# tier4/icp_rust

Hardware: AMD Instinct MI355X
Metric: ICP iterations/sec on 1M-pt 3D pair (higher is better)
Workload: dtype f64

## Files before the change

### icp_rust_amd/csrc/gn_device.hpp

```cpp
#pragma once
#include "common.hpp"

namespace icp {

__device__ __forceinline__ unsigned long long f2k(double v) {
  const unsigned long long u = (unsigned long long)__double_as_longlong(v);
  return (u >> 63) ? ~u : (u | 0x8000000000000000ull);
}
__device__ __forceinline__ double k2f(unsigned long long k) {
  const unsigned long long u = (k >> 63) ? (k & 0x7fffffffffffffffull) : ~k;
  return __longlong_as_double((long long)u);
}

__device__ __forceinline__ int pass_shift(int pass) { return pass < 5 ? 52 - 12 * pass : 0; }
__device__ __forceinline__ int pass_bits(int pass) { return pass < 5 ? 12 : 4; }

__device__ __forceinline__ double huber_rho(double e) {
  const double k = ICP_HUBER_K;
  const double k2 = k * k;
  return (e <= k2) ? e : (2. * k * __dsqrt_rn(e) - k2);
}
__device__ __forceinline__ double huber_drho(double e) {
  const double k = ICP_HUBER_K;
  const double k2 = k * k;
// ... 224 lines not shown
      accumulate_pair<true>(s[u], r0[u], r1[u], T, acc);
    }
  }
}

template <int SCOPE = __HIP_MEMORY_SCOPE_AGENT>
__device__ __forceinline__ void fold_block_sums(const double *partials, int blocks, double *s_tot) {
  double tot[kNSum + 1];
#pragma unroll
  for (int k = 0; k < kNSum + 1; ++k) tot[k] = 0.;
  for (int i = threadIdx.x; i < blocks; i += kReduceThreads) {
    double v[kNSum];
#pragma unroll
    for (int k = 0; k < kNSum; ++k)
      v[k] = __hip_atomic_load(&partials[(size_t)i * (kNSum + 1) + k], __ATOMIC_RELAXED, SCOPE);
#pragma unroll
    for (int k = 0; k < kNSum; ++k) tot[k] = tot[k] + v[k];
  }
  block_reduce_store<kNSum + 1>(tot, s_tot);
}

template <int SCOPE = __HIP_MEMORY_SCOPE_AGENT>
__device__ __forceinline__ void fold_block_sums_lean(const double *partials, int blocks, double *s_tot) {
  __shared__ double sm[kReduceThreads / 64];
  const int t = threadIdx.x;
  for (int q = 0; q < kNSum; ++q) {
    double v[1] = {0.};
    for (int i = t; i < blocks; i += kReduceThreads)
      v[0] = v[0] + __hip_atomic_load(&partials[(size_t)i * (kNSum + 1) + q], __ATOMIC_RELAXED, SCOPE);
    wave_tree<1>(v);
    if ((t & 63) == 0) sm[t >> 6] = v[0];
    __syncthreads();
    if (t == 0) {
      double s = sm[0];
      for (int w = 1; w < kReduceThreads / 64; ++w) s = s + sm[w];
      s_tot[q] = s;
    }
    __syncthreads();
  }
  if (t == 0) s_tot[kNSum] = 0.;
  __syncthreads();
}

constexpr int kFoldH = (kNSum + 1) / 2;
template <int SCOPE = __HIP_MEMORY_SCOPE_AGENT>
__device__ __forceinline__ void fold256_load(const double *partials, int blocks, double (&x)[kFoldH]) {
  static_assert(kReduceThreads == 512 && (kNSum + 1) == 20 && kReduceMaxBlocks <= 256, "two halves of ten sums, one row per thread");
  const int t = threadIdx.x, row = t & 255, half = t >> 8;
#pragma unroll
  for (int k = 0; k < kFoldH; ++k)
    x[k] = (row < blocks && half * kFoldH + k < kNSum)
               ? __hip_atomic_load(&partials[(size_t)row * (kNSum + 1) + half * kFoldH + k], __ATOMIC_RELAXED, SCOPE)
               : 0.;
}
__device__ __forceinline__ void fold256_reduce(const double (&x)[kFoldH], int blocks, double *s_tot) {
  constexpr int H = kFoldH;
  __shared__ double sm[8][H];
  const int t = threadIdx.x, row = t & 255, lane = t & 63, wave = t >> 6;
  double v[H];
#pragma unroll
  for (int k = 0; k < H; ++k) v[k] = 0.;
  if (row < blocks) {
#pragma unroll
    for (int k = 0; k < H; ++k) v[k] = v[k] + x[k];
  }
  wave_tree<H>(v);
  if (lane == 0) {
#pragma unroll
    for (int k = 0; k < H; ++k) sm[wave][k] = v[k];
  }
  __syncthreads();
  if (t < kNSum + 1) {
    const int h = t / H, k = t % H;
    double s = sm[4 * h][k];
    for (int w = 1; w < 4; ++w) s = s + sm[4 * h + w][k];
    s_tot[t] = s + 0.;
  }
}
constexpr int kFoldQ = kFoldH / 2;
template <int SCOPE = __HIP_MEMORY_SCOPE_AGENT>
__device__ __forceinline__ void fold256_half_load(const double *partials, int blocks, int h, double (&x)[kFoldQ]) {
  static_assert(kFoldQ * 2 == kFoldH, "two quarters per half");
  const int t = threadIdx.x, row = t & 255, c0 = h * kFoldH + (t >> 8) * kFoldQ;
#pragma unroll
  for (int k = 0; k < kFoldQ; ++k)
    x[k] = (row < blocks && c0 + k < kNSum)
               ? __hip_atomic_load(&partials[(size_t)row * (kNSum + 1) + c0 + k], __ATOMIC_RELAXED, SCOPE)
               : 0.;
}
__device__ __forceinline__ void fold256_half_reduce(const double (&x)[kFoldQ], int blocks, double *out) {
  constexpr int Q = kFoldQ;
  __shared__ double sm[8][Q];
  const int t = threadIdx.x, row = t & 255, lane = t & 63, wave = t >> 6;
  double v[Q];
#pragma unroll
  for (int k = 0; k < Q; ++k) v[k] = 0.;
  if (row < blocks) {
#pragma unroll
    for (int k = 0; k < Q; ++k) v[k] = v[k] + x[k];
  }
  wave_tree<Q>(v);
  if (lane == 0) {
#pragma unroll
    for (int k = 0; k < Q; ++k) sm[wave][k] = v[k];
  }
  __syncthreads();
  if (t < kFoldH) {
    const int g = t / Q, k = t % Q;
    double s = sm[4 * g][k];
    for (int w = 1; w < 4; ++w) s = s + sm[4 * g + w][k];
    out[t] = s + 0.;
  }
}

template <int SCOPE = __HIP_MEMORY_SCOPE_AGENT>
__device__ __forceinline__ void fold_block_sums_256(const double *partials, int blocks, double *s_tot) {
  double x[kFoldH];
  fold256_load<SCOPE>(partials, blocks, x);
  fold256_reduce(x, blocks, s_tot);
}

template <int SCOPE = __HIP_MEMORY_SCOPE_AGENT>
__device__ __forceinline__ double fold_one_load(const double *partials, int blocks, int q) {
  const int t = threadIdx.x;
  return (t < 256 && t < blocks && q < kNSum) ? __hip_atomic_load(&partials[(size_t)t * (kNSum + 1) + q], __ATOMIC_RELAXED, SCOPE)
                                               : 0.;
}
__device__ __forceinline__ double fold_one_reduce(double x, int blocks, double *sm4) {
  const int t = threadIdx.x, lane = t & 63, wave = t >> 6;
  double v[1] = {0.};
  if (t < 256 && t < blocks) v[0] = v[0] + x;
  wave_tree<1>(v);
  if (t < 256 && lane == 0) sm4[wave] = v[0];
  __syncthreads();
  double s = sm4[0];
  for (int w = 1; w < 4; ++w) s = s + sm4[w];
  return s + 0.;
}
template <int SCOPE = __HIP_MEMORY_SCOPE_AGENT>
__device__ __forceinline__ double fold_one_sum_256(const double *partials, int blocks, int q, double *sm4) {
  const int t = threadIdx.x, lane = t & 63, wave = t >> 6;
  double v[1] = {0.};
  if (t < 256) {
    const double x = (t < blocks && q < kNSum) ? __hip_atomic_load(&partials[(size_t)t * (kNSum + 1) + q], __ATOMIC_RELAXED, SCOPE) : 0.;
    if (t < blocks) v[0] = v[0] + x;
  }
  wave_tree<1>(v);
  if (t < 256 && lane == 0) sm4[wave] = v[0];
  __syncthreads();
  double s = sm4[0];
  for (int w = 1; w < 4; ++w) s = s + sm4[w];
  return s + 0.;
}

__device__ __forceinline__ void publish_folded(const double *s_tot, GnResult *res, unsigned seq, const double (&sig)[2],
                                               const double (&med)[2], int nan_flag, int overflow) {
  if (threadIdx.x < 64) {
    if (threadIdx.x < kNAcc + 1)
      res->acc[threadIdx.x] = threadIdx.x < kNAcc ? combine_sum(s_tot, (int)threadIdx.x, sig) : 0.;
    if (threadIdx.x == kNAcc + 1) {
      res->sigma[0] = sig[0];
      res->sigma[1] = sig[1];
      res->median[0] = med[0];
      res->median[1] = med[1];
    }
    if (threadIdx.x == kNAcc + 2) {
      res->nan_flag = nan_flag;
      res->overflow = overflow;
    }
    asm volatile("s_waitcnt vmcnt(0)" ::: "memory");
    if (threadIdx.x == 0) __hip_atomic_store(&res->seq, seq, __ATOMIC_RELEASE, __HIP_MEMORY_SCOPE_SYSTEM);
// ... 40 lines not shown
```

### icp_rust_amd/csrc/gn_win.hip

```cpp
#include "common.hpp"
#include "gn_device.hpp"
#include "gn_win_device.hpp"
#include "gn_loop.hpp"

namespace icp {


template <bool SUMS, int BATCH = kWinBatch>
__device__ __forceinline__ void win_hist_body(const double2 *__restrict__ a, const double2 *__restrict__ b,
                                              const Pose &T, double *__restrict__ rx, double *__restrict__ ry,
                                              unsigned n, const WinParams &P, uint32_t *whist, WinState *st,
                                              GnScalars *scal, double *partials, int status_cls = -1) {
  __shared__ uint32_t lh[2 * kWinBins];
  if (SUMS && status_cls >= 0 && blockIdx.x == 0 && threadIdx.x < (unsigned)kShardStatusWords)
    whist[2 * kWinBins + threadIdx.x] = (int)threadIdx.x == status_cls ? 1u : 0u;
  double acc[SUMS ? kNSum : 1];
#pragma unroll
  for (int k = 0; k < (SUMS ? kNSum : 1); ++k) acc[k] = 0.;
#ifdef ICP_WIN_DEBUG
  long long wst[6];
  wst[0] = wall_clock64();
#endif
  for (unsigned i = threadIdx.x; i < 2u * kWinBins; i += kWinThreads) lh[i] = 0;
  __syncthreads();
// ... 747 lines not shown
      __hip_atomic_store(&whist[i], 0u, __ATOMIC_RELAXED, __HIP_MEMORY_SCOPE_AGENT);
    fail = fail || got[0] != sel.med_cnt[0] || got[1] != sel.med_cnt[1] || got[2] != sel.ring_cnt[0] ||
           got[3] != sel.ring_cnt[1];
    const unsigned klo = (n - 1) / 2, khi = n / 2;
    if (!fail) {
      unsigned long long key[2][2];
      const double m_lo[2] = {sel.range[0][0], sel.range[1][0]}, m_hi[2] = {sel.range[0][1], sel.range[1][1]};
      const long long mlo[2] = {(long long)klo - sel.med_base[0], (long long)klo - sel.med_base[1]};
      const long long mhi[2] = {(long long)khi - sel.med_base[0], (long long)khi - sel.med_base[1]};
#ifdef ICP_WIN_DEBUG
      fst[3] = wall_clock64();
#endif
      select_n<2, PM>(vm, sel.med_cnt, m_lo, m_hi, mlo, mhi, key, fail);
#ifdef ICP_WIN_DEBUG
      fst[4] = wall_clock64();
#endif
      if (!fail) {
#pragma unroll
        for (int d = 0; d < 2; ++d) {
          med[d] = middle_of(n, key[d][0], key[d][1]);
#pragma unroll
          for (int u = 0; u < PR; ++u) vr[d][u] = fabs(vr[d][u] - med[d]);
        }
        const double r_lo[2] = {sel.range[0][2], sel.range[1][2]}, r_hi[2] = {sel.range[0][3], sel.range[1][3]};
        const long long dlo[2] = {(long long)klo - sel.inner[0], (long long)klo - sel.inner[1]};
        const long long dhi[2] = {(long long)khi - sel.inner[0], (long long)khi - sel.inner[1]};
        select_n<2, PR>(vr, sel.ring_cnt, r_lo, r_hi, dlo, dhi, key, fail);
        if (!fail) {
          sig[0] = ICP_PPF34 * middle_of(n, key[0][0], key[0][1]);
          sig[1] = ICP_PPF34 * middle_of(n, key[1][0], key[1][1]);
        } else {
          med[0] = med[1] = 0.;
        }
      }
    }
  }
  if (tid == 0 && fail) st->fail = 1u;
  asm volatile("s_waitcnt vmcnt(0)" ::: "memory");
  __syncthreads();
  if (ahead && tid == 0) fill_ahead_pose(s_tot, sig, !fail && !nan_flag, outer, ahead, res);
#ifdef ICP_WIN_DEBUG
  fst[5] = wall_clock64();
#endif
  publish_folded(s_tot, res, seq, sig, med, nan_flag, fail ? 2 : 0);
#ifdef ICP_WIN_DEBUG
  asm volatile("s_waitcnt vmcnt(0)" ::: "memory");
  fst[6] = wall_clock64();
  if (tid == 0 && seq % 16 == 5)
    printf("[F last blk %d of %d] compact %lld ticket %lld loads %lld sel1 %lld sel2 %lld publish %lld (x10ns) cnt %u %u %u %u\n", blockIdx.x,
           gridDim.x, fst[1] - fst[0], fst[2] - fst[1], fst[3] - fst[2], fst[4] - fst[3], fst[5] - fst[4], fst[6] - fst[5],
           sel.med_cnt[0], sel.med_cnt[1], sel.ring_cnt[0], sel.ring_cnt[1]);
#endif
}

struct PickLds {
  union {
    struct {
      uint32_t cum[2 * kWinBins];
      uint32_t med[2][kWinCapMed], ring[2][kWinCapRing];
    } g;
    SelectLds<2> sel;
  };
};

struct PickDimLds {
  union {
    struct {
      uint32_t cum[kWinBins];
      double med[kWinCapMed], ring[kWinCapRing];
    } g;
    SelectLds<1> sel;
  };
};

struct WinBins1 {
  unsigned mlo, mhi, a0, b1, i0, i1;
  bool fail;
};
struct WinSel1 {
  unsigned med_base, med_cnt, inner, ring_cnt;
  double range[4];
};

__device__ __forceinline__ WinBins1 win_resolve_dim(const uint32_t *__restrict__ row, unsigned n, const WinDim &w,
                                                    WinState *st, int d, uint32_t *cum, WinSel1 &sel) {
  __shared__ unsigned s_wtot[kReduceThreads / 64];
  __shared__ int s_j[2], s_t[2], s_rng[7];
  __shared__ unsigned s_selu[4];
  __shared__ double s_seld[4];
  constexpr int PER = kWinBins / kReduceThreads, NW = kReduceThreads / 64;
  static_assert(PER == 4, "one 16-byte load per thread");
  const int tid = threadIdx.x, lane = tid & 63, wave = tid >> 6;
  const unsigned klo = (n - 1) / 2, khi = n / 2;
  if (tid < 2) s_j[tid] = -1;
  const uint4 x = reinterpret_cast<const uint4 *>(row)[tid];
  const unsigned v[PER] = {x.x, x.y, x.z, x.w};
  const unsigned tot = (x.x + x.y) + (x.z + x.w);
  const unsigned inc = wave_scan_inclusive(tot);
  if (lane == 63) s_wtot[wave] = inc;
  __syncthreads();
  {
    unsigned wbase = 0;
#pragma unroll
    for (int q = 0; q < NW; ++q) wbase += (q < wave) ? s_wtot[q] : 0u;
    unsigned run = wbase + inc - tot;
#pragma unroll
    for (int i = 0; i < PER; ++i) {
      cum[PER * tid + i] = run;
      if (run <= klo && klo < run + v[i]) s_j[0] = PER * tid + i;
      if (run <= khi && khi < run + v[i]) s_j[1] = PER * tid + i;
      run += v[i];
    }
  }
  __syncthreads();
  WinGeom geo = {};
  if (wave < 2) {
    geo = window_geometry(cum, n, w, s_j[0], s_j[1]);
    const int t = geo.ok ? bracket_search(cum, n, w, geo, wave) : -1;
    if (lane == 0) s_t[wave] = t;
  }
  __syncthreads();
  if (wave == 0) {
    WinRanges R = {};
    unsigned med_base = 0, med_cnt = 0, inner = 0, ring_cnt = 0;
    double range[4] = {0., 0., 0., 0.};
    unsigned counted = 0;
#pragma unroll
    for (int q = 0; q < NW; ++q) counted += s_wtot[q];
    bool ok = counted == n && resolve_window(cum, n, w, geo, s_t[0], s_t[1], R, med_base, med_cnt, inner, ring_cnt, range);
    if (ok)
      ok = R.mlo >= kF1 && R.mhi < kC1 && R.i0 <= R.i1 && R.a0 >= kF0 && R.i0 - 1 < kC0 && R.i1 + 1 >= kF2 &&
           R.b1 <= kWinBins - 2;
    if (lane == 0) {
      s_rng[0] = R.mlo;
      s_rng[1] = R.mhi;
      s_rng[2] = R.a0;
      s_rng[3] = R.b1;
      s_rng[4] = R.i0;
      s_rng[5] = R.i1;
      s_rng[6] = ok ? 0 : 1;
      s_selu[0] = med_base;
      s_selu[1] = med_cnt;
      s_selu[2] = inner;
      s_selu[3] = ring_cnt;
#pragma unroll
      for (int k = 0; k < 4; ++k) s_seld[k] = range[k];
      if (st) {
        st->med_base[d] = med_base;
        st->med_cnt[d] = med_cnt;
        st->ring_inner[d] = inner;
        st->ring_cnt[d] = ring_cnt;
        st->med_lo[d] = range[0];
        st->med_hi[d] = range[1];
        st->ring_lo[d] = range[2];
        st->ring_hi[d] = range[3];
      }
    }
  }
  __syncthreads();
  WinBins1 B;
  B.mlo = (unsigned)s_rng[0];
  B.mhi = (unsigned)s_rng[1];
  B.a0 = (unsigned)s_rng[2];
  B.b1 = (unsigned)s_rng[3];
  B.i0 = (unsigned)s_rng[4];
  B.i1 = (unsigned)s_rng[5];
  B.fail = s_rng[6] != 0;
  sel.med_base = s_selu[0];
  sel.med_cnt = s_selu[1];
  sel.inner = s_selu[2];
  sel.ring_cnt = s_selu[3];
#pragma unroll
  for (int k = 0; k < 4; ++k) sel.range[k] = s_seld[k];
  return B;
}

struct PickArgs {
  unsigned n;
  WinParams P;
  uint32_t *whist;
  WinState *st;
  const double *seg_all;
  const unsigned short *dir_all;
  int segments;
  GnScalars *scal;
  const double *partials;
  int sum_blocks;
  GnResult *res;
  unsigned seq;
  AheadPose *ahead;
  Pose outer;
  WinJoin *join;
};

__device__ __forceinline__ void win_pick_dim_body(const PickArgs &A, const int d, const bool primary, PickDimLds &L) {
  const unsigned n = A.n;
  WinState *const st = A.st;
  const double *__restrict__ seg_all = A.seg_all;
  const unsigned short *__restrict__ dir_all = A.dir_all;
  WinJoin *const J = A.join;
  constexpr int PM = kWinCapMed / kReduceThreads, PR = kWinCapRing / kReduceThreads;
  static_assert(kReduceMaxBlocks * 2 == kReduceThreads, "two threads per segment");
  __shared__ double s_tot[kNSum + 1];
  __shared__ unsigned s_wcnt[kReduceThreads / 64];
  __shared__ int s_last;
  __shared__ unsigned s_pflags;
  __shared__ double s_pms[2];
  const unsigned tid = threadIdx.x;
#ifdef ICP_WIN_DEBUG
  long long pst[10];
  pst[0] = wall_clock64();
  for (int k = 1; k < 10; ++k) pst[k] = pst[0];
#define PSTAMP(k) pst[k] = wall_clock64()
#else
#define PSTAMP(k)
#endif
  const int nan_flag = __hip_atomic_load(&A.scal->nan_flag, __ATOMIC_RELAXED, __HIP_MEMORY_SCOPE_AGENT);
  const unsigned stage_overflow = __hip_atomic_load(&st->stage_overflow, __ATOMIC_RELAXED, __HIP_MEMORY_SCOPE_AGENT);
  WinSel1 sel;
  const WinBins1 R = win_resolve_dim(A.whist + (size_t)d * kWinBins, n, A.P.d[d], primary ? st : nullptr, d, L.g.cum, sel);
  double fx[kFoldQ];
  fold256_half_load(A.partials, A.sum_blocks, d, fx);
  PSTAMP(1);
  const bool fail = R.fail;
  bool bucket_miss = stage_overflow != 0, sel_fail = false;
  double med = 0., sig = 0.;
  {
    const bool usable = !fail && !bucket_miss;
    constexpr int kPickU = 12;
    const unsigned w = tid & (unsigned)(kReduceMaxBlocks - 1), part = tid / (unsigned)kReduceMaxBlocks;
    const unsigned lane = tid & 63u, wave = tid >> 6;
    unsigned p0 = 0, l0 = 0, p1 = 0, l1 = 0;
    if (usable && (int)w < A.segments) {
      const unsigned short *dir = dir_all + (size_t)w * kBktDir;
      if (part == 0) {
        const unsigned fm = word_to_fine(d, R.mlo), len_m = R.mhi - R.mlo + 1u;
        const unsigned m0 = dir[fm], m_end = dir[fm + len_m];
        p0 = m0;
        l0 = m_end - m0;
      } else {
        const unsigned fa = word_to_fine(d, R.a0), fb = word_to_fine(d, R.i1 + 1u);
        const unsigned len_a = R.i0 - R.a0, len_b = R.b1 - R.i1;
        const unsigned a_beg = dir[fa], a_end = dir[fa + len_a], b_beg = dir[fb], b_end = dir[fb + len_b];
        p0 = a_beg;
        l0 = a_end - a_beg;
        p1 = b_beg;
        l1 = b_end - b_beg;
      }
    }
    const unsigned cnt = l0 + l1;
    const unsigned nld = cnt < (unsigned)kBktStage ? cnt : (unsigned)kBktStage;
    const double *const seg = seg_all + (size_t)w * kBktStage;
    auto member = [&](unsigned k) -> unsigned { return k < l0 ? p0 + k : p1 + (k - l0); };
    double own[kPickU];
#pragma unroll
    for (int u = 0; u < kPickU; ++u) {
      const unsigned at = member((unsigned)u);
      own[u] = ((unsigned)u < nld && at < (unsigned)kBktStage) ? seg[at] : 0.;
    }
    const unsigned inc = wave_scan_inclusive(cnt);
    if (lane == 63u) s_wcnt[wave] = inc;
    __syncthreads();
    PSTAMP(2);
    unsigned before = 0, tot_m = 0, tot_r = 0;
    {
      constexpr unsigned HW = kReduceThreads / 64 / 2;
#pragma unroll
      for (unsigned q = 0; q < 2 * HW; ++q) {
        const unsigned x = s_wcnt[q];
        if (q < HW) tot_m += x;
        else tot_r += x;
        before += (q < wave && (q < HW) == (wave < HW)) ? x : 0u;
      }
    }
    if (usable) bucket_miss = tot_m != sel.med_cnt || tot_r != sel.ring_cnt;
    const bool go = usable && !bucket_miss;
    if (go) {
      double *const vals = part ? L.g.ring : L.g.med;
      const unsigned cap = part ? (unsigned)kWinCapRing : (unsigned)kWinCapMed;
      const unsigned off = before + inc - cnt;
#pragma unroll
      for (int u = 0; u < kPickU; ++u)
        if ((unsigned)u < nld && off + (unsigned)u < cap) vals[off + (unsigned)u] = own[u];
      for (unsigned k = kPickU; k < nld; ++k) {
        const unsigned at = member(k);
        if (at < (unsigned)kBktStage && off + k < cap) vals[off + k] = seg[at];
      }
    }
    __syncthreads();
    double vm[1][PM], vr[1][PR];
#pragma unroll
    for (int u = 0; u < PM; ++u) {
      const unsigned e = tid + u * kReduceThreads;
      vm[0][u] = (go && e < sel.med_cnt) ? L.g.med[e] : 0.;
    }
#pragma unroll
    for (int u = 0; u < PR; ++u) {
      const unsigned e = tid + u * kReduceThreads;
      vr[0][u] = (go && e < sel.ring_cnt) ? L.g.ring[e] : 0.;
    }
    {
      unsigned long long *row = reinterpret_cast<unsigned long long *>(A.whist + (size_t)d * kWinBins);
#pragma unroll
      for (int u = 0; u < kWinBins / 2 / kReduceThreads; ++u)
        __hip_atomic_store(&row[tid + u * kReduceThreads], 0ull, __ATOMIC_RELAXED, __HIP_MEMORY_SCOPE_AGENT);
// ... 2 lines not shown
    __syncthreads();
    PSTAMP(3);
    const unsigned klo = (n - 1) / 2, khi = n / 2;
    if (go) {
      unsigned long long key[1][2];
      const unsigned cm[1] = {sel.med_cnt}, cr[1] = {sel.ring_cnt};
      const double m_lo[1] = {sel.range[0]}, m_hi[1] = {sel.range[1]};
      const long long mlo[1] = {(long long)klo - sel.med_base}, mhi[1] = {(long long)khi - sel.med_base};
      select_n_lds<1, PM>(vm, cm, m_lo, m_hi, mlo, mhi, key, sel_fail, L.sel);
      PSTAMP(4);
      if (!sel_fail) {
        med = middle_of(n, key[0][0], key[0][1]);
#pragma unroll
        for (int u = 0; u < PR; ++u) vr[0][u] = fabs(vr[0][u] - med);
        const double r_lo[1] = {sel.range[2]}, r_hi[1] = {sel.range[3]};
        const long long dlo[1] = {(long long)klo - sel.inner}, dhi[1] = {(long long)khi - sel.inner};
        select_n_lds<1, PR>(vr, cr, r_lo, r_hi, dlo, dhi, key, sel_fail, L.sel);
        PSTAMP(5);
        if (!sel_fail) sig = ICP_PPF34 * middle_of(n, key[0][0], key[0][1]);
      }
    }
  }
  const unsigned flags = (fail ? 1u : 0u) | (bucket_miss ? 2u : 0u) | (sel_fail ? 4u : 0u);
  WinJoinDim *const mine = &J->dim[d];
  if (tid < (unsigned)kFoldH) __hip_atomic_store(&mine->tot[tid], s_tot[d * kFoldH + tid], __ATOMIC_RELAXED, __HIP_MEMORY_SCOPE_AGENT);
  if (tid == 64) {
    __hip_atomic_store(&mine->med, med, __ATOMIC_RELAXED, __HIP_MEMORY_SCOPE_AGENT);
    __hip_atomic_store(&mine->sig, sig, __ATOMIC_RELAXED, __HIP_MEMORY_SCOPE_AGENT);
    __hip_atomic_store(&mine->flags, flags, __ATOMIC_RELAXED, __HIP_MEMORY_SCOPE_AGENT);
  }
  asm volatile("s_waitcnt vmcnt(0)" ::: "memory");
  __syncthreads();
  PSTAMP(6);
  if (tid == 0)
    s_last = (int)(__hip_atomic_fetch_add(&J->ticket, 1u, __ATOMIC_RELAXED, __HIP_MEMORY_SCOPE_AGENT) & 1u);
  __syncthreads();
  if (!s_last) {
#ifdef ICP_WIN_DEBUG
    if (tid == 0 && A.seq % 16 == 5)
      printf("[P%d first] resolve %lld dir+scan %lld place+fold %lld sel1 %lld sel2 %lld store %lld (x10ns) cnt %u %u\n", d,
             pst[1] - pst[0], pst[2] - pst[1], pst[3] - pst[2], pst[4] - pst[3], pst[5] - pst[4], pst[6] - pst[5],
             sel.med_cnt, sel.ring_cnt);
#endif
    return;
  }
  const int o = 1 - d;
  const WinJoinDim *const other = &J->dim[o];
  static_assert(offsetof(WinJoinDim, tot) == 16 && offsetof(WinJoinDim, flags) == 96, "words of the record");
  if (tid < 13) {
    const unsigned long long x =
        __hip_atomic_load(reinterpret_cast<const unsigned long long *>(other) + tid, __ATOMIC_RELAXED, __HIP_MEMORY_SCOPE_AGENT);
    if (tid < 2) s_pms[tid] = __longlong_as_double((long long)x);
    else if (tid < 12) s_tot[o * kFoldH + (tid - 2)] = __longlong_as_double((long long)x);
    else s_pflags = (unsigned)x;
  }
  __syncthreads();
  PSTAMP(7);
  const unsigned all = flags | s_pflags;
  const bool any_fail = (all & 1u) != 0, any_bucket = (all & 2u) != 0;
  const bool failed = any_fail || (!any_bucket && (all & 4u) != 0);
  const bool missed = failed || any_bucket;
  const double m_me = missed ? 0. : med, s_me = missed ? 0. : sig, m_ot = missed ? 0. : s_pms[0], s_ot = missed ? 0. : s_pms[1];
  const double med2[2] = {d ? m_ot : m_me, d ? m_me : m_ot}, sig2[2] = {d ? s_ot : s_me, d ? s_me : s_ot};
  if (tid == 0) {
    if (missed) st->fail = 1u;
    else if (primary) st->fail = 0u;
    if (stage_overflow) __hip_atomic_store(&st->stage_overflow, 0u, __ATOMIC_RELAXED, __HIP_MEMORY_SCOPE_AGENT);
  }
  const int overflow = missed ? (failed ? 2 : 3) : 0;
  GnResult *const res = A.res;
  if (A.ahead) {
    if (tid == 0) fill_ahead_pose(s_tot, sig2, !missed && !nan_flag, A.outer, A.ahead, res);
    publish_values<1>(s_tot, res, sig2, med2, nan_flag, overflow);
    PSTAMP(8);
    __syncthreads();
    publish_seq(res, A.seq);
  } else {
    PSTAMP(8);
    publish_folded(s_tot, res, A.seq, sig2, med2, nan_flag, overflow);
  }
#ifdef ICP_WIN_DEBUG
  asm volatile("s_waitcnt vmcnt(0)" ::: "memory");
  PSTAMP(9);
  if (tid == 0 && A.seq % 16 == 5)
    printf("[P%d last] resolve %lld dir+scan %lld place+fold %lld sel1 %lld sel2 %lld store %lld ticket+loads %lld ahead %lld "
           "publish %lld (x10ns) cnt %u %u\n", d, pst[1] - pst[0], pst[2] - pst[1], pst[3] - pst[2], pst[4] - pst[3],
           pst[5] - pst[4], pst[6] - pst[5], pst[7] - pst[6], pst[8] - pst[7], pst[9] - pst[8], sel.med_cnt, sel.ring_cnt);
#endif
#undef PSTAMP
}

__global__ __launch_bounds__(kReduceThreads) void k_win_pick(PickArgs A) {
  __shared__ PickDimLds L;
  win_pick_dim_body(A, (int)blockIdx.x, true, L);
}

__global__ __launch_bounds__(kWinThreads, 4) void k_win_hist_sums_bkt2(HistBktArgs A, HistBktArgs B) {
  __shared__ HistBktLds S;
  const unsigned half = gridDim.x >> 1;
  if (blockIdx.x < half) win_hist_sums_bkt_body(A, blockIdx.x, half, S);
  else win_hist_sums_bkt_body(B, blockIdx.x - half, half, S);
}
struct PickPairArgs {
  PickArgs e[2];
};
__global__ __launch_bounds__(kReduceThreads) void k_win_pick2(PickPairArgs X) {
  __shared__ PickDimLds L;
  const unsigned second = blockIdx.x >> 1;
  win_pick_dim_body(X.e[second], (int)(blockIdx.x & 1u), second == 0u, L);
}

namespace {
constexpr long long kPipeTimeoutTicks = 300000000;
__device__ __forceinline__ void pst_u32(unsigned *p, unsigned v) { __hip_atomic_store(p, v, __ATOMIC_RELAXED, __HIP_MEMORY_SCOPE_SYSTEM); }
__device__ __forceinline__ void pst_f64(double *p, double v) { __hip_atomic_store(p, v, __ATOMIC_RELAXED, __HIP_MEMORY_SCOPE_SYSTEM); }
__device__ __forceinline__ unsigned pld_u32(const unsigned *p) { return __hip_atomic_load(p, __ATOMIC_RELAXED, __HIP_MEMORY_SCOPE_SYSTEM); }
__device__ __forceinline__ double pld_f64(const double *p) { return __hip_atomic_load(p, __ATOMIC_RELAXED, __HIP_MEMORY_SCOPE_SYSTEM); }

__device__ __forceinline__ bool pipe_poll(const unsigned long long *words, int count, unsigned gen, LoopInbox *const *box, int W,
                                          LoopInbox *me, unsigned *payload_or) {
  __shared__ int s_pok;
  __shared__ unsigned s_ppay;
  if (threadIdx.x < 64) {
    const int lane = (int)threadIdx.x;
    unsigned long long seen = 0;
    int ok = 1;
    const long long t0 = wall_clock64();
    for (;;) {
      bool here = true;
      if (lane < count) {
        seen = __hip_atomic_load(&words[lane], __ATOMIC_RELAXED, __HIP_MEMORY_SCOPE_SYSTEM);
        here = (int)((unsigned)seen - gen) >= 0;
      }
      if (__all(here)) break;
      int stop = 0;
      if (lane == 0) {
        if (pld_u32(&me->abort[0]) != 0u) stop = 1;
        else if (wall_clock64() - t0 > kPipeTimeoutTicks) {
          for (int q = 0; q < W; ++q) pst_u32(&box[q]->abort[0], 1u);
          stop = 1;
        }
      }
      if (__builtin_amdgcn_readfirstlane(stop)) {
        ok = 0;
        break;
      }
      __builtin_amdgcn_s_sleep(1);
    }
    unsigned pay = lane < count ? (unsigned)(seen >> 32) : 0u;
#pragma unroll
    for (int off = 32; off >= 1; off >>= 1) pay |= (unsigned)__shfl_xor((int)pay, off);
    if (lane == 0) {
      s_pok = ok;
      s_ppay = pay;
    }
  }
  __syncthreads();
  *payload_or = s_ppay;
  return s_pok != 0;
}
}

constexpr int kPipeFuse = 8;
struct PickRank {
  uint32_t *whist;
  WinState *st;
  const double *seg_all;
  const unsigned short *dir_all;
  GnScalars *scal;
  const double *partials;
// ... 694 lines not shown
```

### icp_rust_amd/csrc/gn_win_device.hpp

```cpp
#pragma once
#include "common.hpp"
#include "gn_device.hpp"

namespace icp {

constexpr int kWinThreads = 512;
constexpr int kWinBatch = 4;
#ifndef ICP_SELECT_DIRECT
#define ICP_SELECT_DIRECT 256
#endif
constexpr int kSubBins = 1024;
constexpr int kSmallCap = 1024;
constexpr size_t kWinMinN = 1u << 12;
constexpr size_t kWinMaxN = 1u << 22;

constexpr int kF0 = 1, kC0 = kF0 + kWinFine, kF1 = kC0 + kWinCoarse, kC1 = kF1 + kWinFine, kF2 = kC1 + kWinCoarse;
static_assert(kF2 + kWinFine == kWinBins - 1, "bin layout");

__device__ __forceinline__ unsigned region_bin(double off, double scale, int first, int count) {
  const unsigned k = (unsigned)(off * scale);
  return (unsigned)first + (k < (unsigned)count ? k : (unsigned)(count - 1));
}

__device__ __forceinline__ unsigned wbin(double r, const WinDim &w) {
  if (!(r >= w.x[0])) return 0u;
  if (r >= w.x[5]) return (unsigned)(kWinBins - 1);
  if (r < w.x[1]) return region_bin(r - w.x[0], w.sf, kF0, kWinFine);
  if (r < w.x[2]) return region_bin(r - w.x[1], w.sc, kC0, kWinCoarse);
  if (r < w.x[3]) return region_bin(r - w.x[2], w.sf, kF1, kWinFine);
  if (r < w.x[4]) return region_bin(r - w.x[3], w.sc, kC1, kWinCoarse);
  return region_bin(r - w.x[4], w.sf, kF2, kWinFine);
}

__device__ __forceinline__ unsigned wbin_cold(double r, const WinDim &w) {
  const bool g1 = r >= w.x[1], g2 = r >= w.x[2], g3 = r >= w.x[3], g4 = r >= w.x[4];
  const double base = g4 ? w.x[4] : (g3 ? w.x[3] : (g2 ? w.x[2] : (g1 ? w.x[1] : w.x[0])));
  const bool coarse = g1 != g2 || g3 != g4;
  const int first = g4 ? kF2 : (g3 ? kC1 : (g2 ? kF1 : (g1 ? kC0 : kF0)));
  const bool inside = r >= w.x[0] && !(r >= w.x[5]);
  const double off = inside ? r - base : 0.;
  const unsigned j = region_bin(off, coarse ? w.sc : w.sf, first, coarse ? kWinCoarse : kWinFine);
  if (!(r >= w.x[0])) return 0u;
  return r >= w.x[5] ? (unsigned)(kWinBins - 1) : j;
}

struct WinRegion {
  double base, scale;
  unsigned first, last;
  unsigned pad[2];
};
static_assert(sizeof(WinRegion) == 32, "one ds_read_b128 + one ds_read_b64");
__device__ __forceinline__ void win_region_table(const WinDim &w, WinRegion *tab, int r) {
  const bool coarse = r & 1;
  WinRegion e;
  e.base = w.x[r];
  e.scale = coarse ? w.sc : w.sf;
  e.first = (unsigned)(r == 0 ? kF0 : r == 1 ? kC0 : r == 2 ? kF1 : r == 3 ? kC1 : kF2);
  e.last = (unsigned)((coarse ? kWinCoarse : kWinFine) - 1);
  e.pad[0] = e.pad[1] = 0u;
  tab[r] = e;
}
__device__ __forceinline__ unsigned wbin_tab(double r, const WinDim &w, const WinRegion *tab, bool &below, bool &above,
                                             bool &fine) {
  below = !(r >= w.x[0]);
  above = r >= w.x[5];
  const unsigned reg = (unsigned)(r >= w.x[1]) + (unsigned)(r >= w.x[2]) + (unsigned)(r >= w.x[3]) + (unsigned)(r >= w.x[4]);
  const WinRegion e = tab[reg];
  const unsigned k = (unsigned)((r - e.base) * e.scale);
  fine = !(reg & 1u) & !below & !above;
  const unsigned j = e.first + (k < e.last ? k : e.last);
  return below ? 0u : (above ? (unsigned)(kWinBins - 1) : j);
}

__device__ __forceinline__ bool fine_bin(unsigned j) {
  return (j - (unsigned)kF0 < (unsigned)kWinFine) | (j - (unsigned)kF1 < (unsigned)kWinFine) |
         (j - (unsigned)kF2 < (unsigned)kWinFine);
}

__device__ __forceinline__ double wedge(int j, const WinDim &w) {
  if (j >= kWinBins - 1) return w.x[5];
  const bool g1 = j >= kC0, g2 = j >= kF1, g3 = j >= kC1, g4 = j >= kF2;
  const double base = g4 ? w.x[4] : (g3 ? w.x[3] : (g2 ? w.x[2] : (g1 ? w.x[1] : w.x[0])));
  const int first = g4 ? kF2 : (g3 ? kC1 : (g2 ? kF1 : (g1 ? kC0 : kF0)));
  const bool coarse = g1 != g2 || g3 != g4;
  return base + (double)(j - first) / (coarse ? w.sc : w.sf);
}

template <typename F>
__device__ __forceinline__ int wave_last_true(int lo, int hi, F &&pred) {
  const int lane = threadIdx.x & 63;
  int best = lo - 1;
  while (lo <= hi) {
    const int step = (hi - lo + 64) >> 6;
    const int t = lo + lane * step;
    const bool ok = t <= hi && pred(t);
    const int cnt = __popcll(__ballot(ok));
    if (cnt == 0) break;
    best = lo + (cnt - 1) * step;
    const int nhi = best + step - 1 < hi ? best + step - 1 : hi;
    lo = best + 1;
    hi = nhi;
  }
  return best;
}

struct WinRanges {
  int mlo, mhi;
  int a0, b1;
  int i0, i1;
};

struct WinGeom {
  int jlo, jhi;
  double mL, mU, fine, q;
  int tmax;
  bool ok;
};

__device__ __forceinline__ WinGeom window_geometry(const uint32_t *c, unsigned n, const WinDim &w, int jlo_known = -1,
                                                   int jhi_known = -1) {
  auto C = [&](int j) -> unsigned { return j >= kWinBins ? n : c[j]; };
  const unsigned klo = (n - 1) / 2, khi = n / 2;
  WinGeom g;
  if (jlo_known >= 0 && jhi_known >= 0) {
    g.jlo = jlo_known;
    g.jhi = jhi_known;
  } else {
    g.jlo = wave_last_true(0, kWinBins - 1, [&](int j) { return c[j] <= klo; });
    g.jhi = (C(g.jlo + 1) > khi) ? g.jlo : wave_last_true(0, kWinBins - 1, [&](int j) { return c[j] <= khi; });
  }
  g.ok = !(g.jlo < 1 || g.jhi > kWinBins - 2);
  g.mL = g.ok ? wedge(g.jlo, w) : 0.;
  g.mU = g.ok ? wedge(g.jhi + 1, w) : 0.;
  g.fine = 1. / w.sf;
  g.q = 0.25 * g.fine;
  g.tmax = (int)((w.x[5] - w.x[0]) * w.sf) + 2;
  return g;
}

__device__ __forceinline__ void inside_bins(const WinGeom &g, const WinDim &w, double d, int &s, int &e) {
  s = (int)wbin_cold(g.mU - d + g.q, w) + 1;
  e = (int)wbin_cold(g.mL + d - g.q, w);
}
__device__ __forceinline__ void possible_bins(const WinGeom &g, const WinDim &w, double d, int &s, int &e) {
  s = (int)wbin_cold(g.mL - d - g.q, w);
  e = (int)wbin_cold(g.mU + d + g.q, w) + 1;
}

__device__ __forceinline__ int bracket_search(const uint32_t *c, unsigned n, const WinDim &w, const WinGeom &g,
                                              int role) {
  auto C = [&](int j) -> unsigned { return j >= kWinBins ? n : c[j]; };
  const unsigned klo = (n - 1) / 2, khi = n / 2;
  if (role == 0)
    return wave_last_true(0, g.tmax, [&](int t) {
      int s, e;
      possible_bins(g, w, (double)t * g.fine, s, e);
      return C(e) - C(s) <= klo;
    });
  return wave_last_true(0, g.tmax, [&](int t) {
           int s, e;
           inside_bins(g, w, (double)t * g.fine, s, e);
           return (s < e ? C(e) - C(s) : 0u) <= khi;
         }) + 1;
}

__device__ __forceinline__ bool resolve_window(const uint32_t *c, unsigned n, const WinDim &w, const WinGeom &g,
                                               int t1, int t2, WinRanges &R, unsigned &med_base,
                                               unsigned &med_cnt, unsigned &inner, unsigned &ring_cnt,
                                               double (&range)[4]) {
  auto C = [&](int j) -> unsigned { return j >= kWinBins ? n : c[j]; };
  if (!g.ok || t1 < 0 || t2 > g.tmax) return false;
  const int jlo = g.jlo, jhi = g.jhi;
  const double fine = g.fine, q = g.q;
  int is, ie, ps, pe;
  inside_bins(g, w, (double)t1 * fine - 2. * q, is, ie);
  possible_bins(g, w, (double)t2 * fine + 2. * q, ps, pe);
  if (ps < 1 || pe > kWinBins - 1) return false;
  R.mlo = jlo;
  R.mhi = jhi;
  R.a0 = ps;
  R.b1 = pe - 1;
  if (is < ie) {
    R.i0 = is;
    R.i1 = ie - 1;
    inner = C(ie) - C(is);
  } else {
    R.i0 = 1;
    R.i1 = 0;
    inner = 0u;
  }
  med_base = c[jlo];
  med_cnt = C(jhi + 1) - c[jlo];
  ring_cnt = (C(pe) - C(ps)) - inner;
  range[0] = g.mL;
  range[1] = g.mU;
  range[2] = t1 > 0 ? (double)(t1 - 1) * fine : 0.;
  range[3] = (double)(t2 + 1) * fine;
  return med_cnt <= (unsigned)kWinCapMed && ring_cnt <= (unsigned)kWinCapRing;
}

__device__ __forceinline__ unsigned block_excl_scan(unsigned v, unsigned *total) {
  __shared__ unsigned s_w[kReduceThreads / 64];
  const int lane = threadIdx.x & 63, wave = threadIdx.x >> 6;
  const unsigned s = wave_scan_inclusive(v);
  if (lane == 63) s_w[wave] = s;
  __syncthreads();
  unsigned before = 0, all = 0;
#pragma unroll
  for (int w = 0; w < kReduceThreads / 64; ++w) {
    const unsigned x = s_w[w];
    all += x;
    before += (w < wave) ? x : 0u;
  }
  __syncthreads();
  *total = all;
  return before + s - v;
}

template <int ND>
struct SelectLds {
  unsigned hist[ND][kSubBins];
  unsigned long long small_keys[ND][kSmallCap];
  unsigned long long out[ND][2];
  unsigned nsmall[ND], sb[ND][2], below[ND];
};

template <int ND, int NV, int DIRECT = ICP_SELECT_DIRECT>
__device__ __forceinline__ void select_n_lds(const double (&v)[ND][NV], const unsigned (&cnt)[ND],
                                             const double (&lo)[ND], const double (&hi)[ND],
                                             const long long (&rlo)[ND], const long long (&rhi)[ND],
                                             unsigned long long (&out)[ND][2], bool &fail, SelectLds<ND> &S) {
  static_assert(ND == 1 || ND == 2, "one or two lists");
  static_assert(kSubBins == 2 * kReduceThreads, "geometry");
  auto &s_hist = S.hist;
  auto &s_small = S.small_keys;
  auto &s_nsmall = S.nsmall;
  auto &s_sb = S.sb;
  auto &s_below = S.below;
  auto &s_out = S.out;
  const unsigned tid = threadIdx.x;
#pragma unroll
  for (int d = 0; d < ND; ++d) out[d][0] = out[d][1] = 0;
#pragma unroll
  for (int d = 0; d < ND; ++d)
    if (rlo[d] < 0 || rhi[d] >= (long long)cnt[d] || rhi[d] < rlo[d] || cnt[d] > 0xffffu) fail = true;
  if (fail) return;
// ... 185 lines not shown
```

Measured before the change: 10330.

## Parallelize window bracket search across workgroup and hoist histogram row load

Replaces the per-wave bracket search, where two waves each ran a serial wave_last_true search and wave 0 alone resolved the window, with a workgroup-wide coarse sampling pass (256 samples per role via ballot), then a single-wave fine pass. Every thread now computes resolve_window redundantly, which removes two barriers and the shared-memory broadcast of results. The histogram row load is moved earlier so it overlaps with the partials fold load. The fold load reads unconditionally from a clamped row address and masks afterwards, so the loads can be issued without branches. The cost is redundant computation in all threads and some extra logic, plus debug timestamps.

```diff
diff --git a/icp_rust_amd/csrc/gn_device.hpp b/icp_rust_amd/csrc/gn_device.hpp
--- a/icp_rust_amd/csrc/gn_device.hpp
+++ b/icp_rust_amd/csrc/gn_device.hpp
@@ -330,11 +330,13 @@
 __device__ __forceinline__ void fold256_half_load(const double *partials, int blocks, int h, double (&x)[kFoldQ]) {
   static_assert(kFoldQ * 2 == kFoldH, "two quarters per half");
   const int t = threadIdx.x, row = t & 255, c0 = h * kFoldH + (t >> 8) * kFoldQ;
-#pragma unroll
-  for (int k = 0; k < kFoldQ; ++k)
-    x[k] = (row < blocks && c0 + k < kNSum)
-               ? __hip_atomic_load(&partials[(size_t)row * (kNSum + 1) + c0 + k], __ATOMIC_RELAXED, SCOPE)
-               : 0.;
+  static_assert(2 * kFoldH == kNSum + 1, "the last column read is the padding word");
+  const double *const p = partials + (size_t)(row < blocks ? row : 0) * (kNSum + 1) + c0;
+  double v[kFoldQ];
+#pragma unroll
+  for (int k = 0; k < kFoldQ; ++k) v[k] = __hip_atomic_load(&p[k], __ATOMIC_RELAXED, SCOPE);
+#pragma unroll
+  for (int k = 0; k < kFoldQ; ++k) x[k] = (row < blocks && c0 + k < kNSum) ? v[k] : 0.;
 }
 __device__ __forceinline__ void fold256_half_reduce(const double (&x)[kFoldQ], int blocks, double *out) {
   constexpr int Q = kFoldQ;
diff --git a/icp_rust_amd/csrc/gn_win.hip b/icp_rust_amd/csrc/gn_win.hip
--- a/icp_rust_amd/csrc/gn_win.hip
+++ b/icp_rust_amd/csrc/gn_win.hip
@@ -853,27 +853,44 @@
   double range[4];
 };
 
-__device__ __forceinline__ WinBins1 win_resolve_dim(const uint32_t *__restrict__ row, unsigned n, const WinDim &w,
-                                                    WinState *st, int d, uint32_t *cum, WinSel1 &sel) {
-  __shared__ unsigned s_wtot[kReduceThreads / 64];
-  __shared__ int s_j[2], s_t[2], s_rng[7];
-  __shared__ unsigned s_selu[4];
-  __shared__ double s_seld[4];
+#ifdef ICP_WIN_DEBUG
+__device__ long long g_rdbg[4][8];
+#define RSTAMP(k)                                         \
+  do {                                                    \
+    asm volatile("s_waitcnt vmcnt(0) lgkmcnt(0)" ::: "memory"); \
+    if (threadIdx.x == 0) g_rdbg[blockIdx.x][k] = wall_clock64(); \
+  } while (0)
+#else
+#define RSTAMP(k)
+#endif
+__device__ __forceinline__ WinBins1 win_resolve_dim(const uint4 x, unsigned n, const WinDim &w, WinState *st, int d,
+                                                    uint32_t *cum, WinSel1 &sel) {
+  __shared__ unsigned s_wtot[kReduceThreads / 64], s_bcnt[kReduceThreads / 64];
+  __shared__ int s_j[2];
   constexpr int PER = kWinBins / kReduceThreads, NW = kReduceThreads / 64;
   static_assert(PER == 4, "one 16-byte load per thread");
   const int tid = threadIdx.x, lane = tid & 63, wave = tid >> 6;
   const unsigned klo = (n - 1) / 2, khi = n / 2;
   if (tid < 2) s_j[tid] = -1;
-  const uint4 x = reinterpret_cast<const uint4 *>(row)[tid];
+#ifdef ICP_WIN_DEBUG
+  if (tid < 8) g_rdbg[blockIdx.x][tid] = 0;
+  RSTAMP(0);
+#endif
   const unsigned v[PER] = {x.x, x.y, x.z, x.w};
   const unsigned tot = (x.x + x.y) + (x.z + x.w);
   const unsigned inc = wave_scan_inclusive(tot);
   if (lane == 63) s_wtot[wave] = inc;
   __syncthreads();
+  RSTAMP(1);
+  unsigned counted = 0;
   {
     unsigned wbase = 0;
 #pragma unroll
-    for (int q = 0; q < NW; ++q) wbase += (q < wave) ? s_wtot[q] : 0u;
+    for (int q = 0; q < NW; ++q) {
+      const unsigned x = s_wtot[q];
+      counted += x;
+      wbase += (q < wave) ? x : 0u;
+    }
     unsigned run = wbase + inc - tot;
 #pragma unroll
     for (int i = 0; i < PER; ++i) {
@@ -884,65 +901,44 @@
     }
   }
   __syncthreads();
-  WinGeom geo = {};
-  if (wave < 2) {
-    geo = window_geometry(cum, n, w, s_j[0], s_j[1]);
-    const int t = geo.ok ? bracket_search(cum, n, w, geo, wave) : -1;
-    if (lane == 0) s_t[wave] = t;
-  }
-  __syncthreads();
-  if (wave == 0) {
-    WinRanges R = {};
-    unsigned med_base = 0, med_cnt = 0, inner = 0, ring_cnt = 0;
-    double range[4] = {0., 0., 0., 0.};
-    unsigned counted = 0;
-#pragma unroll
-    for (int q = 0; q < NW; ++q) counted += s_wtot[q];
-    bool ok = counted == n && resolve_window(cum, n, w, geo, s_t[0], s_t[1], R, med_base, med_cnt, inner, ring_cnt, range);
-    if (ok)
-      ok = R.mlo >= kF1 && R.mhi < kC1 && R.i0 <= R.i1 && R.a0 >= kF0 && R.i0 - 1 < kC0 && R.i1 + 1 >= kF2 &&
-           R.b1 <= kWinBins - 2;
-    if (lane == 0) {
-      s_rng[0] = R.mlo;
-      s_rng[1] = R.mhi;
-      s_rng[2] = R.a0;
-      s_rng[3] = R.b1;
-      s_rng[4] = R.i0;
-      s_rng[5] = R.i1;
-      s_rng[6] = ok ? 0 : 1;
-      s_selu[0] = med_base;
-      s_selu[1] = med_cnt;
-      s_selu[2] = inner;
-      s_selu[3] = ring_cnt;
-#pragma unroll
-      for (int k = 0; k < 4; ++k) s_seld[k] = range[k];
-      if (st) {
-        st->med_base[d] = med_base;
-        st->med_cnt[d] = med_cnt;
-        st->ring_inner[d] = inner;
-        st->ring_cnt[d] = ring_cnt;
-        st->med_lo[d] = range[0];
-        st->med_hi[d] = range[1];
-        st->ring_lo[d] = range[2];
-        st->ring_hi[d] = range[3];
-      }
-    }
-  }
-  __syncthreads();
+  RSTAMP(2);
+  const WinGeom geo = window_geometry(cum, n, w, s_j[0], s_j[1]);
+  RSTAMP(3);
+  int t1, t2;
+  bracket_search_wg(cum, n, w, geo, s_bcnt, t1, t2);
+  RSTAMP(4);
+  WinRanges R = {};
+  unsigned med_base = 0, med_cnt = 0, inner = 0, ring_cnt = 0;
+  double range[4] = {0., 0., 0., 0.};
+  bool ok = counted == n && resolve_window(cum, n, w, geo, t1, t2, R, med_base, med_cnt, inner, ring_cnt, range);
+  if (ok)
+    ok = R.mlo >= kF1 && R.mhi < kC1 && R.i0 <= R.i1 && R.a0 >= kF0 && R.i0 - 1 < kC0 && R.i1 + 1 >= kF2 &&
+         R.b1 <= kWinBins - 2;
+  RSTAMP(5);
+  if (st && tid == 0) {
+    st->med_base[d] = med_base;
+    st->med_cnt[d] = med_cnt;
+    st->ring_inner[d] = inner;
+    st->ring_cnt[d] = ring_cnt;
+    st->med_lo[d] = range[0];
+    st->med_hi[d] = range[1];
+    st->ring_lo[d] = range[2];
+    st->ring_hi[d] = range[3];
+  }
   WinBins1 B;
-  B.mlo = (unsigned)s_rng[0];
-  B.mhi = (unsigned)s_rng[1];
-  B.a0 = (unsigned)s_rng[2];
-  B.b1 = (unsigned)s_rng[3];
-  B.i0 = (unsigned)s_rng[4];
-  B.i1 = (unsigned)s_rng[5];
-  B.fail = s_rng[6] != 0;
-  sel.med_base = s_selu[0];
-  sel.med_cnt = s_selu[1];
-  sel.inner = s_selu[2];
-  sel.ring_cnt = s_selu[3];
-#pragma unroll
-  for (int k = 0; k < 4; ++k) sel.range[k] = s_seld[k];
+  B.mlo = (unsigned)R.mlo;
+  B.mhi = (unsigned)R.mhi;
+  B.a0 = (unsigned)R.a0;
+  B.b1 = (unsigned)R.b1;
+  B.i0 = (unsigned)R.i0;
+  B.i1 = (unsigned)R.i1;
+  B.fail = !ok;
+  sel.med_base = med_base;
+  sel.med_cnt = med_cnt;
+  sel.inner = inner;
+  sel.ring_cnt = ring_cnt;
+#pragma unroll
+  for (int k = 0; k < 4; ++k) sel.range[k] = range[k];
   return B;
 }
 
@@ -986,12 +982,13 @@
 #else
 #define PSTAMP(k)
 #endif
+  const uint4 hrow = reinterpret_cast<const uint4 *>(A.whist + (size_t)d * kWinBins)[tid];
   const int nan_flag = __hip_atomic_load(&A.scal->nan_flag, __ATOMIC_RELAXED, __HIP_MEMORY_SCOPE_AGENT);
   const unsigned stage_overflow = __hip_atomic_load(&st->stage_overflow, __ATOMIC_RELAXED, __HIP_MEMORY_SCOPE_AGENT);
-  WinSel1 sel;
-  const WinBins1 R = win_resolve_dim(A.whist + (size_t)d * kWinBins, n, A.P.d[d], primary ? st : nullptr, d, L.g.cum, sel);
   double fx[kFoldQ];
   fold256_half_load(A.partials, A.sum_blocks, d, fx);
+  WinSel1 sel;
+  const WinBins1 R = win_resolve_dim(hrow, n, A.P.d[d], primary ? st : nullptr, d, L.g.cum, sel);
   PSTAMP(1);
   const bool fail = R.fail;
   bool bucket_miss = stage_overflow != 0, sel_fail = false;
@@ -1160,10 +1157,15 @@
 #ifdef ICP_WIN_DEBUG
   asm volatile("s_waitcnt vmcnt(0)" ::: "memory");
   PSTAMP(9);
-  if (tid == 0 && A.seq % 16 == 5)
+  if (tid == 0 && A.seq % 16 == 5) {
+    printf("[R%d] loads %lld row+scan %lld cum %lld geometry %lld bracket %lld resolve_window %lld (x10ns)\n", d,
+           g_rdbg[blockIdx.x][0] - pst[0], g_rdbg[blockIdx.x][1] - g_rdbg[blockIdx.x][0], g_rdbg[blockIdx.x][2] - g_rdbg[blockIdx.x][1],
+           g_rdbg[blockIdx.x][3] - g_rdbg[blockIdx.x][2], g_rdbg[blockIdx.x][4] - g_rdbg[blockIdx.x][3],
+           g_rdbg[blockIdx.x][5] - g_rdbg[blockIdx.x][4]);
     printf("[P%d last] resolve %lld dir+scan %lld place+fold %lld sel1 %lld sel2 %lld store %lld ticket+loads %lld ahead %lld "
            "publish %lld (x10ns) cnt %u %u\n", d, pst[1] - pst[0], pst[2] - pst[1], pst[3] - pst[2], pst[4] - pst[3],
            pst[5] - pst[4], pst[6] - pst[5], pst[7] - pst[6], pst[8] - pst[7], pst[9] - pst[8], sel.med_cnt, sel.ring_cnt);
+  }
 #endif
 #undef PSTAMP
 }
diff --git a/icp_rust_amd/csrc/gn_win_device.hpp b/icp_rust_amd/csrc/gn_win_device.hpp
--- a/icp_rust_amd/csrc/gn_win_device.hpp
+++ b/icp_rust_amd/csrc/gn_win_device.hpp
@@ -39,7 +39,8 @@
   const int first = g4 ? kF2 : (g3 ? kC1 : (g2 ? kF1 : (g1 ? kC0 : kF0)));
   const bool inside = r >= w.x[0] && !(r >= w.x[5]);
   const double off = inside ? r - base : 0.;
-  const unsigned j = region_bin(off, coarse ? w.sc : w.sf, first, coarse ? kWinCoarse : kWinFine);
+  const double sf = w.sf, sc = w.sc;
+  const unsigned j = region_bin(off, coarse ? sc : sf, first, coarse ? kWinCoarse : kWinFine);
   if (!(r >= w.x[0])) return 0u;
   return r >= w.x[5] ? (unsigned)(kWinBins - 1) : j;
 }
@@ -162,6 +163,55 @@
            inside_bins(g, w, (double)t * g.fine, s, e);
            return (s < e ? C(e) - C(s) : 0u) <= khi;
          }) + 1;
+}
+
+__device__ __forceinline__ bool bracket_pred(const uint32_t *c, unsigned n, const WinDim &w, const WinGeom &g, int role,
+                                             int t) {
+  const unsigned klo = (n - 1) / 2, khi = n / 2;
+  const double mL = g.mL, mU = g.mU, q = g.q;
+  const double d = (double)t * g.fine, sq = role ? q : -q;
+  const int s = (int)wbin_cold(((role ? mU : mL) - d) + sq, w) + role;
+  const int e = (int)wbin_cold(((role ? mL : mU) + d) - sq, w) + 1 - role;
+  const unsigned cs = c[s < kWinBins ? s : kWinBins - 1], ce = c[e < kWinBins ? e : kWinBins - 1];
+  const unsigned Cs = s >= kWinBins ? n : cs, Ce = e >= kWinBins ? n : ce;
+  return (s < e ? Ce - Cs : 0u) <= (role ? khi : klo);
+}
+
+__device__ __forceinline__ void bracket_search_wg(const uint32_t *c, unsigned n, const WinDim &w, const WinGeom &g,
+                                                  unsigned *s_cnt, int &t1, int &t2) {
+  static_assert(kReduceThreads == 512, "four waves per role");
+  const int tid = threadIdx.x, lane = tid & 63, wave = tid >> 6;
+  const int step = (g.tmax + 256) >> 8;
+  {
+    const int t = (tid & 255) * step;
+    const bool p = g.ok && t <= g.tmax && bracket_pred(c, n, w, g, wave >> 2, t);
+    const unsigned cnt = (unsigned)__popcll(__ballot(p));
+    if (lane == 0) s_cnt[wave] = cnt;
+  }
+  __syncthreads();
+  int lo[2], hi[2];
+#pragma unroll
+  for (int r = 0; r < 2; ++r) {
+    const int cnt = (int)((s_cnt[4 * r] + s_cnt[4 * r + 1]) + (s_cnt[4 * r + 2] + s_cnt[4 * r + 3]));
+    const int best = (cnt - 1) * step;
+    lo[r] = cnt ? best + 1 : 0;
+    hi[r] = cnt ? (best + step - 1 < g.tmax ? best + step - 1 : g.tmax) : -1;
+  }
+  if (step <= 33) {
+    const int r = lane >> 5, t = (r ? lo[1] : lo[0]) + (lane & 31);
+    const bool p = t <= (r ? hi[1] : hi[0]) && bracket_pred(c, n, w, g, r, t);
+    const unsigned long long m = __ballot(p);
+    t1 = lo[0] - 1 + __popc((unsigned)m);
+    t2 = lo[1] - 1 + __popc((unsigned)(m >> 32)) + 1;
+  } else {
+    t1 = t2 = 0;
+#pragma unroll 1
+    for (int r = 0; r < 2; ++r) {
+      const int v = wave_last_true(r ? lo[1] : lo[0], r ? hi[1] : hi[0], [&](int t) { return bracket_pred(c, n, w, g, r, t); });
+      if (r) t2 = v + 1;
+      else t1 = v;
+    }
+  }
 }
 
 __device__ __forceinline__ bool resolve_window(const uint32_t *c, unsigned n, const WinDim &w, const WinGeom &g,
```

Measured after the change: 10440 (median of 6 runs). No clear change (+1.1%).
